# jzombie/rust-llkv

Measured on AMD Instinct MI355X. Metric: rows/sec + HBM GB/s, TPC-H Q1/Q6 SF10 at 1/2/4/8 MI355X, higher is better.
Workload: dtype f64

## Files before the change

### rust-llkv_amd/csrc/fused_scan.hip.h

```cpp
#pragma once

#ifndef __HIPCC_RTC__
#include <hip/hip_runtime.h>
#include <stdint.h>
#endif

#include "scan_params.h"
#include "planvalue_rules.h"

namespace llkv {

__device__ __forceinline__ uint64_t lane_identity(int op) {
  switch (op) {
  case OP_MIN_I64: return 0x7FFFFFFFFFFFFFFFull;
  case OP_MAX_I64: return 0x8000000000000000ull;
  default: return 0ull;
  }
}

__device__ __forceinline__ uint64_t lane_combine(int op, uint64_t a, uint64_t b) {
  const uint64_t fadd = (uint64_t)__double_as_longlong(__longlong_as_double((long long)a) + __longlong_as_double((long long)b));
  const uint64_t iadd = a + b;
  const bool lt = (int64_t)b < (int64_t)a;
  const uint64_t imin = lt ? b : a;
  const uint64_t imax = (int64_t)b > (int64_t)a ? b : a;
  const uint64_t umax = b > a ? b : a;
  return op == OP_ADD_F64 ? fadd : op == OP_ADD_I64 ? iadd : op == OP_MIN_I64 ? imin : op == OP_MAX_I64 ? imax : umax;
}

template <int OP> __device__ __forceinline__ uint64_t lane_combine_s(uint64_t a, uint64_t b) {
  if constexpr (OP == OP_ADD_F64) return (uint64_t)__double_as_longlong(__longlong_as_double((long long)a) + __longlong_as_double((long long)b));
  else if constexpr (OP == OP_ADD_I64) return a + b;
  else if constexpr (OP == OP_MIN_I64) return (int64_t)b < (int64_t)a ? b : a;
  else if constexpr (OP == OP_MAX_I64) return (int64_t)b > (int64_t)a ? b : a;
  else return b > a ? b : a;
}

template <int OP> constexpr uint64_t lane_identity_s() {
  return OP == OP_MIN_I64 ? 0x7FFFFFFFFFFFFFFFull : OP == OP_MAX_I64 ? 0x8000000000000000ull : 0ull;
}

struct I32 { using T = int32_t; static constexpr int W = 4; static constexpr bool is_float = false; };
struct U32 { using T = uint32_t; static constexpr int W = 4; static constexpr bool is_float = false; };
struct F32 { using T = float; static constexpr int W = 4; static constexpr bool is_float = true; };
struct I64 { using T = int64_t; static constexpr int W = 8; static constexpr bool is_float = false; };
struct U64 { using T = uint64_t; static constexpr int W = 8; static constexpr bool is_float = false; };
struct F64 { using T = double; static constexpr int W = 8; static constexpr bool is_float = true; };
struct I128 { using T = __int128; static constexpr int W = 16; static constexpr bool is_float = false; };
struct U8 { using T = uint8_t; static constexpr int W = 1; static constexpr bool is_float = false; };
template <class Ty, int N_> struct D8 { using T = typename Ty::T; static constexpr int W = 1; static constexpr int N = N_; static constexpr bool is_float = Ty::is_float; };

template <class... Ts> struct Cols { static constexpr int N = sizeof...(Ts); };

template <int I, class L> struct ColAt;
template <int I, class T0, class... Ts> struct ColAt<I, Cols<T0, Ts...>> { using type = typename ColAt<I - 1, Cols<Ts...>>::type; };
template <class T0, class... Ts> struct ColAt<0, Cols<T0, Ts...>> { using type = T0; };

struct Loaded {
  uint32_t w[kMaxCols][4];
};

#ifndef LLKV_NT_LOADS
#define LLKV_NT_LOADS 1
#endif
template <class V> __device__ __forceinline__ V stream_load(const V *ptr) {
#if LLKV_NT_LOADS
  return __builtin_nontemporal_load(ptr);
#else
  return *ptr;
#endif
}

template <class Ty> __device__ __forceinline__ void load_pair(const void *base, uint64_t row, uint32_t (&w)[4]) {
  if constexpr (Ty::W == 8) {
    typedef uint32_t v4u __attribute__((ext_vector_type(4)));
    const v4u v = stream_load(reinterpret_cast<const v4u *>(static_cast<const char *>(base) + row * 8));
    w[0] = v.x; w[1] = v.y; w[2] = v.z; w[3] = v.w;
  } else if constexpr (Ty::W == 4) {
    typedef uint32_t v2u __attribute__((ext_vector_type(2)));
    const v2u v = stream_load(reinterpret_cast<const v2u *>(static_cast<const char *>(base) + row * 4));
    w[0] = v.x; w[1] = v.y;
  } else {
    w[0] = stream_load(reinterpret_cast<const uint16_t *>(static_cast<const char *>(base) + row));
  }
}

template <class Ty> __device__ __forceinline__ void load_quad(const void *base, uint64_t row, uint32_t (&w)[4]) {
  static_assert(Ty::W <= 4, "four rows of an 8-byte column do not fit a column's registers");
  if constexpr (Ty::W == 4) {
    typedef uint32_t v4u __attribute__((ext_vector_type(4)));
    const v4u v = stream_load(reinterpret_cast<const v4u *>(static_cast<const char *>(base) + row * 4));
    w[0] = v.x; w[1] = v.y; w[2] = v.z; w[3] = v.w;
  } else {
    w[0] = stream_load(reinterpret_cast<const uint32_t *>(static_cast<const char *>(base) + row));
  }
}
template <class CL, int LO, int HI> __device__ __forceinline__ void load_quad_range(const ScanParams &p, uint64_t row, Loaded &ld) {
  if constexpr (LO < HI && LO < CL::N) {
    load_quad<typename ColAt<LO, CL>::type>(p.col[LO], row, ld.w[LO]);
    load_quad_range<CL, LO + 1, HI>(p, row, ld);
  }
}
template <class CL, int LO, int HI> constexpr bool cols_narrow() {
  if constexpr (LO < HI && LO < CL::N) return ColAt<LO, CL>::type::W <= 4 && ColAt<LO, CL>::type::W != 2 && cols_narrow<CL, LO + 1, HI>();
  else return true;
}

template <class CL, int I = 0> __device__ __forceinline__ void load_all(const ScanParams &p, uint64_t row, Loaded &ld) {
  if constexpr (I < CL::N) {
    load_pair<typename ColAt<I, CL>::type>(p.col[I], row, ld.w[I]);
    load_all<CL, I + 1>(p, row, ld);
  }
}

template <class CL, int LO, int HI> __device__ __forceinline__ void load_range(const ScanParams &p, uint64_t row, Loaded &ld) {
  if constexpr (LO < HI && LO < CL::N) {
    load_pair<typename ColAt<LO, CL>::type>(p.col[LO], row, ld.w[LO]);
    load_range<CL, LO + 1, HI>(p, row, ld);
  }
}

template <class Ty> struct CodedSize { static constexpr int N = 0; };
template <class Ty, int M> struct CodedSize<D8<Ty, M>> {
  static_assert(M >= 1 && M <= 256 && (M & (M - 1)) == 0 && Ty::W == 8, "a decode table has a power of two ≤ 256 of 8-byte entries");
  static constexpr int N = M;
};
template <class CL, int LO, int HI> constexpr int coded_entries() {
  if constexpr (LO < HI && LO < CL::N) return CodedSize<typename ColAt<LO, CL>::type>::N + coded_entries<CL, LO + 1, HI>();
  else return 0;
}
template <int NT> struct ValueTables {
  static __device__ __forceinline__ uint64_t *lds() { __shared__ uint64_t t[NT]; return t; }
};
template <> struct ValueTables<0> {
  static __device__ __forceinline__ uint64_t *lds() { return nullptr; }
};
template <class CL> __device__ __forceinline__ const uint64_t *stage_value_tables(const ScanParams &p) {
  constexpr int NT = coded_entries<CL, 0, CL::N>();
  uint64_t *t = ValueTables<NT>::lds();
  if constexpr (NT > 0) {
    for (uint32_t i = threadIdx.x; i < (uint32_t)NT; i += blockDim.x) t[i] = p.value_tables[i];
    __syncthreads();
  }
  return t;
}
template <class CL, int LO, int HI> __device__ __forceinline__ void decode_range(const uint64_t *vtab, Loaded &ld) {
  if constexpr (LO < HI && LO < CL::N) {
    constexpr int n = CodedSize<typename ColAt<LO, CL>::type>::N;
    if constexpr (n > 0) {
      const uint64_t *t = vtab + coded_entries<CL, 0, LO>();
      const uint32_t codes = ld.w[LO][0];
      const uint64_t a = t[codes & (uint32_t)(n - 1)], b = t[(codes >> 8) & (uint32_t)(n - 1)];
      ld.w[LO][0] = (uint32_t)a; ld.w[LO][1] = (uint32_t)(a >> 32);
      ld.w[LO][2] = (uint32_t)b; ld.w[LO][3] = (uint32_t)(b >> 32);
    }
    decode_range<CL, LO + 1, HI>(vtab, ld);
  }
}

struct Ctx {
  const ScanParams &p;
  const Loaded &ld;
  uint32_t err;
  uint64_t row;
  uint32_t perr;
  uint64_t dval;
  uint32_t dhead;

  template <class Ty> __device__ __forceinline__ typename Ty::T get(int s, int j) const {
    if constexpr (Ty::W == 8) {
      const uint64_t bits = ((uint64_t)ld.w[s][2 * j + 1] << 32) | ld.w[s][2 * j];
      if constexpr (Ty::is_float) return __longlong_as_double((long long)bits);
      else return (typename Ty::T)bits;
    } else if constexpr (Ty::W == 4) {
      if constexpr (Ty::is_float) return __uint_as_float(ld.w[s][j]);
      else return (typename Ty::T)ld.w[s][j];
    } else {
      return (uint8_t)((ld.w[s][0] >> (8 * j)) & 0xffu);
    }
  }
};

template <int S, class Ty> struct Col {
  using Type = Ty;
  static __device__ __forceinline__ typename Ty::T eval(Ctx &c, int j) { return c.get<Ty>(S, j); }
  static __device__ __forceinline__ bool valid(Ctx &, int) { return true; }
};
template <int S, class Ty, int SV> struct ColN {
  using Type = Ty;
  static __device__ __forceinline__ typename Ty::T eval(Ctx &c, int j) { return c.get<Ty>(S, j); }
  static __device__ __forceinline__ bool valid(Ctx &c, int j) { return c.get<U8>(SV, j) != 0; }
};
template <int K> struct LitI {
  using Type = I64;
  static __device__ __forceinline__ int64_t eval(Ctx &c, int) { return c.p.lit_i[K]; }
  static __device__ __forceinline__ bool valid(Ctx &, int) { return true; }
};
template <int K> struct LitU {
  using Type = U64;
  static __device__ __forceinline__ uint64_t eval(Ctx &c, int) { return (uint64_t)c.p.lit_i[K]; }
  static __device__ __forceinline__ bool valid(Ctx &, int) { return true; }
};
template <int K> struct LitF {
  using Type = F64;
  static __device__ __forceinline__ double eval(Ctx &c, int) { return c.p.lit_f[K]; }
  static __device__ __forceinline__ bool valid(Ctx &, int) { return true; }
};
template <int S> struct DictNum {
  using Type = F64;
  static __device__ __forceinline__ double eval(Ctx &c, int j) { return c.p.dict_num[S * 256 + (int)c.get<U8>(S, j)]; }
  static __device__ __forceinline__ bool valid(Ctx &, int) { return true; }
};
template <class E> struct ToF64 {
  using Type = F64;
  static __device__ __forceinline__ double eval(Ctx &c, int j) { return (double)E::eval(c, j); }
  static __device__ __forceinline__ bool valid(Ctx &c, int j) { return E::valid(c, j); }
};
template <class E> struct Widen128 {
  using Type = I128;
  static __device__ __forceinline__ __int128 eval(Ctx &c, int j) { return (__int128)(int64_t)E::eval(c, j); }
  static __device__ __forceinline__ bool valid(Ctx &c, int j) { return E::valid(c, j); }
};
template <int SLO, int SHI> struct Join128 {
  using Type = I128;
  static __device__ __forceinline__ __int128 eval(Ctx &c, int j) { return ((__int128)c.get<I64>(SHI, j) << 64) | (__int128)(unsigned __int128)c.get<U64>(SLO, j); }
  static __device__ __forceinline__ bool valid(Ctx &, int) { return true; }
};
template <class E> struct ToI64 {
  using Type = I64;
  static __device__ __forceinline__ int64_t eval(Ctx &c, int j) { return (int64_t)E::eval(c, j); }
  static __device__ __forceinline__ bool valid(Ctx &c, int j) { return E::valid(c, j); }
};

__device__ __forceinline__ int64_t f64_as_i64_sat(double x) {
  if (x != x) return 0;
  if (x >= 9223372036854775808.0) return 0x7FFFFFFFFFFFFFFFll;
  if (x <= -9223372036854775808.0) return (int64_t)0x8000000000000000ull;
  return (int64_t)x;
}

#ifndef LLKV_FIRST_ONLY_MODE
#define LLKV_FIRST_ONLY_MODE 0
#endif
enum BinKind : int { B_ADD = 1, B_SUB = 2, B_MUL = 3, B_REM = 4 };
constexpr uint32_t kErrOverflow = 1u, kErrDivZero = 2u;

__device__ __forceinline__ double f64_result_as_sse2(double r, double a, double b) {
  if (r == r) return r;
  const long long quiet = 0x0008000000000000ll;
  if (a != a) return __longlong_as_double(__double_as_longlong(a) | quiet);
  if (b != b) return __longlong_as_double(__double_as_longlong(b) | quiet);
  return __longlong_as_double((long long)0xFFF8000000000000ull);
}

template <int OP, class L, class R, int EXACT_NAN = 0> struct Bin {
  using Type = typename L::Type;
  static __device__ __forceinline__ bool valid(Ctx &c, int j) { return L::valid(c, j) & R::valid(c, j); }
  static __device__ __forceinline__ typename Type::T eval(Ctx &c, int j) {
    const auto a = L::eval(c, j);
    const auto b = R::eval(c, j);
    if constexpr (Type::is_float) {
      double r;
      if constexpr (OP == B_ADD) r = a + b;
      else if constexpr (OP == B_SUB) r = a - b;
      else if constexpr (OP == B_MUL) r = a * b;
      else r = fmod(a, b);
      if constexpr (EXACT_NAN) return f64_result_as_sse2(r, a, b);
      else return r;
    } else if constexpr (OP == B_REM) {
      const bool ok = valid(c, j);
      const int64_t x = (int64_t)a, y = (int64_t)b;
      const bool zero = y == 0;
      c.err = max(c.err, (ok & zero) ? kErrDivZero : 0u);
      return (zero | (y == -1)) ? 0 : x % y;
    } else {
      int64_t z;
      bool o;
      if constexpr (OP == B_ADD) o = __builtin_add_overflow((int64_t)a, (int64_t)b, &z);
      else if constexpr (OP == B_SUB) o = __builtin_sub_overflow((int64_t)a, (int64_t)b, &z);
      else o = __builtin_mul_overflow((int64_t)a, (int64_t)b, &z);
      c.err = max(c.err, (o & valid(c, j)) ? kErrOverflow : 0u);
      return z;
    }
  }
};
template <class E, int SIGNED> struct Fit32 {
  using Type = I64;
  static __device__ __forceinline__ bool valid(Ctx &c, int j) { return E::valid(c, j); }
  static __device__ __forceinline__ int64_t eval(Ctx &c, int j) {
    const int64_t z = (int64_t)E::eval(c, j);
    const bool fits = SIGNED ? (z >= -2147483648ll && z <= 2147483647ll) : (z >= 0 && z <= 4294967295ll);
    c.err = max(c.err, (!fits & E::valid(c, j)) ? kErrOverflow : 0u);
    return z;
  }
};
template <class E, class T32> struct Narrow32 {
  using Type = T32;
  static __device__ __forceinline__ bool valid(Ctx &c, int j) { return E::valid(c, j); }
  static __device__ __forceinline__ typename T32::T eval(Ctx &c, int j) { return (typename T32::T)E::eval(c, j); }
};
template <class L, class R> using Add = Bin<B_ADD, L, R>;
template <class L, class R> using Sub = Bin<B_SUB, L, R>;
template <class L, class R> using Mul = Bin<B_MUL, L, R>;

template <class L, class R, int EXACT_NAN = 0> struct Div {
  using Type = typename L::Type;
  static __device__ __forceinline__ bool nonzero(typename Type::T b) {
    if constexpr (Type::is_float) return __double_as_longlong(b) != 0;
    else return b != 0;
// ... 729 lines not shown
            const int op = ops.v[gg * K + k];
            const uint64_t x = sel ? contrib[k] : lane_identity(op);
            acc[gg][k] = lane_combine(op, acc[gg][k], x);
          }
        }
      }
    }
  }

  const uint32_t slot = tid + (tid >> 4);
  const uint32_t ri = tid >> 4;
  const uint32_t rq = tid & 15;
#pragma unroll
  for (int base = 0; base < LANES; base += kRedBatch) {
#pragma unroll
    for (int i = 0; i < kRedBatch; ++i) {
      const int lane = base + i;
      if (lane < LANES) {
        uint64_t v;
        if (lane == NG * K) v = err;
        else v = acc[lane / K][lane % K];
        red[i][slot] = v;
      }
    }
    __syncthreads();
    const int lane = base + (int)ri;
    if (lane < LANES) {
      const int op = ops.v[lane];
      const uint32_t seg = rq * 17;
      uint64_t v = red[ri][seg];
#pragma unroll
      for (int e = 1; e < 16; ++e) v = lane_combine(op, v, red[ri][seg + e]);
#pragma unroll
      for (int off = 8; off >= 1; off >>= 1) {
        const uint32_t lo = __shfl_xor((uint32_t)v, off, 16);
        const uint32_t hi = __shfl_xor((uint32_t)(v >> 32), off, 16);
        const uint64_t o = ((uint64_t)hi << 32) | lo;
        v = (rq & off) ? lane_combine(op, o, v) : lane_combine(op, v, o);
      }
      if (rq == 0) publish_partial(p, lane, v, tile, p.n_tiles);
    }
    __syncthreads();
  }
  }
}


template <int OP> __device__ __forceinline__ void lds_accumulate(uint64_t *slot, uint64_t x) {
  if constexpr (OP == OP_ADD_F64)
    (void)__hip_atomic_fetch_add(reinterpret_cast<double *>(slot), __longlong_as_double((long long)x), __ATOMIC_RELAXED, __HIP_MEMORY_SCOPE_WORKGROUP);
  else if constexpr (OP == OP_ADD_I64)
    (void)__hip_atomic_fetch_add(reinterpret_cast<unsigned long long *>(slot), (unsigned long long)x, __ATOMIC_RELAXED, __HIP_MEMORY_SCOPE_WORKGROUP);
  else if constexpr (OP == OP_MIN_I64)
    (void)__hip_atomic_fetch_min(reinterpret_cast<long long *>(slot), (long long)x, __ATOMIC_RELAXED, __HIP_MEMORY_SCOPE_WORKGROUP);
  else if constexpr (OP == OP_MAX_I64)
    (void)__hip_atomic_fetch_max(reinterpret_cast<long long *>(slot), (long long)x, __ATOMIC_RELAXED, __HIP_MEMORY_SCOPE_WORKGROUP);
  else
    (void)__hip_atomic_fetch_max(reinterpret_cast<unsigned long long *>(slot), (unsigned long long)x, __ATOMIC_RELAXED, __HIP_MEMORY_SCOPE_WORKGROUP);
}

template <class P, int K0 = 0> __device__ __forceinline__ void lds_accumulate_row(uint64_t *group_base, const uint64_t *contrib, uint32_t gid, uint64_t *seen) {
  if constexpr (K0 < P::K) {
    if constexpr (plan_lane_first_only<P>(K0)) {
      constexpr int i = plan_first_only_index<P>(K0);
      const uint64_t bit = 1ull << gid;
      if (!(seen[i] & bit) && contrib[K0] != lane_identity_s<plan_lane_op<P>(K0)>()) {
        lds_accumulate<plan_lane_op<P>(K0)>(group_base + K0 * kBlock, contrib[K0]);
        seen[i] |= bit;
      }
    } else {
      lds_accumulate<plan_lane_op<P>(K0)>(group_base + K0 * kBlock, contrib[K0]);
    }
    lds_accumulate_row<P, K0 + 1>(group_base, contrib, gid, seen);
  }
}

__device__ __forceinline__ void wave_lds_sync() {
  __builtin_amdgcn_fence(__ATOMIC_RELEASE, "wavefront");
  __builtin_amdgcn_wave_barrier();
  __builtin_amdgcn_fence(__ATOMIC_ACQUIRE, "wavefront");
}

__device__ __forceinline__ TileDesc load_tile_desc(const TileDesc *tiles, uint32_t i) {
  typedef const __attribute__((address_space(4))) uint64_t *ConstU64;
  ConstU64 q = (ConstU64)(unsigned long long)(tiles + i);
  TileDesc d;
  d.dev_row = q[0];
  d.logical_row = q[1];
  const uint64_t w = q[2];
  d.rows = (uint32_t)w;
  d.octant = (uint32_t)(w >> 32);
  return d;
}

constexpr int kLdsParts = kBlock / 64;

template <class P, int OP> struct OpSlots {
  int n;
  int v[P::K];
  constexpr OpSlots() : n(0), v{} {
    for (int k = 0; k < P::K; ++k)
      if (plan_lane_op<P>(k) == OP) v[n++] = k;
  }
};

template <class P, int OP>
__device__ __forceinline__ void wave_reduce_class(const ScanParams &p, const uint64_t (*acc)[kBlock], uint32_t wave, uint32_t li, uint32_t sq, uint32_t part, uint32_t n_parts) {
  constexpr OpSlots<P, OP> cls{};
  if constexpr (cls.n > 0) {
    constexpr int total = P::NG * cls.n;
#pragma unroll 1
    for (int base = 0; base < total; base += 16) {
      const int idx = base + (int)li;
      if (idx < total) {
        const int g = idx / cls.n, j = idx % cls.n;
        int k = cls.v[0];
#pragma unroll
        for (int t = 1; t < cls.n; ++t) k = j == t ? cls.v[t] : k;
        const int lane = g * P::K + k;
        const uint64_t *seg = &acc[lane][wave * 64 + sq * 16];
        uint64_t x[16];
#pragma unroll
        for (int e = 0; e < 16; ++e) x[e] = seg[(li + e) & 15];
        uint64_t v = x[0];
#pragma unroll
        for (int e = 1; e < 16; ++e) v = lane_combine_s<OP>(v, x[e]);
#pragma unroll
        for (int off = 2; off >= 1; off >>= 1) {
          const uint32_t lo = __shfl_xor((uint32_t)v, off, 4);
          const uint32_t hi = __shfl_xor((uint32_t)(v >> 32), off, 4);
          const uint64_t o = ((uint64_t)hi << 32) | lo;
          v = (sq & off) ? lane_combine_s<OP>(o, v) : lane_combine_s<OP>(v, o);
        }
        if (sq == 0) publish_partial(p, lane, v, part, n_parts);
      }
    }
  }
}

template <class P>
__device__ __forceinline__ void wave_reduce_image(const ScanParams &p, const uint64_t (*acc)[kBlock], uint32_t wave, uint32_t wl, uint32_t part, uint32_t n_parts, uint32_t err) {
  const uint32_t li = wl >> 2, sq = wl & 3;
  wave_lds_sync();
  wave_reduce_class<P, OP_ADD_F64>(p, acc, wave, li, sq, part, n_parts);
  wave_reduce_class<P, OP_ADD_I64>(p, acc, wave, li, sq, part, n_parts);
  wave_reduce_class<P, OP_MIN_I64>(p, acc, wave, li, sq, part, n_parts);
  wave_reduce_class<P, OP_MAX_I64>(p, acc, wave, li, sq, part, n_parts);
  wave_reduce_class<P, OP_MAX_U64>(p, acc, wave, li, sq, part, n_parts);
  const uint32_t wave_err = (__builtin_amdgcn_ballot_w64((err & 1u) != 0) ? 1u : 0u) | (__builtin_amdgcn_ballot_w64((err & 2u) != 0) ? 2u : 0u);
  if (wl == 0) publish_partial(p, P::NG * P::K, wave_err, part, n_parts);
  wave_lds_sync();
}

template <class P> __device__ __forceinline__ void fused_scan_body_lds(const ScanParams &p) {
  constexpr int NG = P::NG, K = P::K, U = P::U;
  constexpr LaneOpTable<P> ops{};
  __shared__ uint64_t acc[NG * K][kBlock];

  const uint32_t tid = threadIdx.x, wave = tid >> 6, wl = tid & 63;
  piggyback_fold<P>(p);

  uint32_t tile = (uint32_t)((uint64_t)blockIdx.x * p.n_tiles / gridDim.x);
  const uint32_t tile_end = (uint32_t)((uint64_t)(blockIdx.x + 1) * p.n_tiles / gridDim.x);
  if (tile >= tile_end) return;
  const uint64_t *vtab = stage_value_tables<typename P::ColList>(p);
  const uint32_t n_parts = p.n_tiles * kLdsParts;
#pragma unroll
  for (int l = 0; l < NG * K; ++l) acc[l][tid] = lane_identity(ops.v[l]);
  uint32_t err = 0, done_err = 0, done_tile = 0;
  constexpr int n_first_only = plan_first_only_index<P>(K);
  static_assert(n_first_only == 0 || NG <= 64, "the first-only masks hold one bit per group");
  uint64_t seen[n_first_only > 0 ? n_first_only : 1] = {};
  bool fresh = false;

  TileDesc td = load_tile_desc(p.tiles, tile);
  TileDesc td_next = load_tile_desc(p.tiles, tile + 1 < tile_end ? tile + 1 : tile);
  uint32_t nsteps = (td.rows + kStepRows - 1) / kStepRows;
  uint32_t s = 0;
  for (;;) {
    Loaded ld[U];
#pragma unroll
    for (int u = 0; u < U; ++u) load_all<typename P::ColList>(p, td.dev_row + (uint64_t)(s + u) * kStepRows + (uint64_t)tid * kRowsPerThread, ld[u]);
    if (fresh) {
      wave_reduce_image<P>(p, acc, wave, wl, done_tile * kLdsParts + wave, n_parts, done_err);
#pragma unroll
      for (int l = 0; l < NG * K; ++l) acc[l][tid] = lane_identity(ops.v[l]);
#pragma unroll
      for (int i = 0; i < (n_first_only > 0 ? n_first_only : 1); ++i) seen[i] = 0;
      fresh = false;
    }
#pragma unroll
    for (int u = 0; u < U; ++u) {
      decode_range<typename P::ColList, 0, P::ColList::N>(vtab, ld[u]);
      const uint32_t row0 = (s + u) * kStepRows + tid * kRowsPerThread;
#pragma unroll
      for (int j = 0; j < kRowsPerThread; ++j) {
        Ctx c{p, ld[u], 0u, td.logical_row + row0 + j};
        const bool in_tile = (row0 + j) < td.rows;
        const bool pass = in_tile & P::Pred::eval(c, j);
        uint32_t gid = P::KeyT::gid(c, j);
        gid = gid < (uint32_t)NG ? gid : 0u;
        uint64_t contrib[K];
        contrib[0] = 1;
        if constexpr (P::first) contrib[1] = c.row;
        AggOps<typename P::AggT>::contrib(c, j, contrib + P::BASE);
        err |= (pass ? c.err : 0u) | (in_tile ? c.perr : 0u);
        if (pass) lds_accumulate_row<P>(&acc[gid * K][tid], contrib, gid, seen);
      }
    }
    s += U;
    if (s >= nsteps) {
      done_tile = tile;
      done_err = err;
      err = 0;
      fresh = true;
      if (++tile >= tile_end) break;
      td = td_next;
      nsteps = (td.rows + kStepRows - 1) / kStepRows;
      s = 0;
      if (tile + 1 < tile_end) td_next = load_tile_desc(p.tiles, tile + 1);
    }
  }
  wave_reduce_image<P>(p, acc, wave, wl, done_tile * kLdsParts + wave, n_parts, done_err);
}

constexpr int kImgBlock = 1024;
constexpr int kImgStepRows = kImgBlock * kRowsPerThread;

constexpr int image_replicas(int cells, int cell_bytes = 8) {
  int r = 1;
  while (r < 32 && (long)(2 * r) * cells * cell_bytes <= 64 * 1024) r *= 2;
  return r;
}
template <bool NARROW> struct ImageCell { using T = uint64_t; };
template <> struct ImageCell<true> { using T = uint32_t; };
template <int OP> __device__ __forceinline__ void lds_accumulate(uint32_t *slot, uint64_t x) {
  static_assert(OP == OP_ADD_I64 || OP == OP_MIN_I64, "4-byte image cells hold counts, bounded integer sums and first rows");
  if constexpr (OP == OP_ADD_I64) (void)__hip_atomic_fetch_add(slot, (uint32_t)x, __ATOMIC_RELAXED, __HIP_MEMORY_SCOPE_WORKGROUP);
  else (void)__hip_atomic_fetch_min(slot, (uint32_t)x, __ATOMIC_RELAXED, __HIP_MEMORY_SCOPE_WORKGROUP);
}
template <class P, int NGS, int K0 = 0, class Cell> __device__ __forceinline__ void image_accumulate_row(Cell *img, uint32_t gid, const uint64_t *contrib) {
  if constexpr (K0 < P::K) {
    lds_accumulate<plan_lane_op<P>(K0)>(img + K0 * NGS + gid, contrib[K0]);
    image_accumulate_row<P, NGS, K0 + 1>(img, gid, contrib);
  }
}

template <class P> __device__ __forceinline__ void image_scan_body(const ScanParams &p) {
  constexpr int K = P::K, U = P::U;
  constexpr int NG = (P::NG + P::PASSES - 1) / P::PASSES;
  using Cell = typename ImageCell<P::CELL32>::T;
  constexpr int R = image_replicas(K * NG, (int)sizeof(Cell));
  __shared__ Cell img_all[R * K * NG];
  __shared__ uint32_t block_err;

  const uint32_t tid = threadIdx.x;
  Cell *img = img_all + (tid % (uint32_t)R) * (uint32_t)(K * NG);
  for (uint32_t i = tid; i < (uint32_t)(R * K * NG); i += kImgBlock) {
    const int op = plan_lane_op<P>((int)((i % (uint32_t)(K * NG)) / NG));
    if constexpr (P::CELL32) img_all[i] = op == OP_MIN_I64 ? 0xFFFFFFFFu : 0u;
    else img_all[i] = lane_identity(op);
  }
  if (tid == 0) block_err = 0;
  const uint64_t *vtab = stage_value_tables<typename P::ColList>(p);
  __syncthreads();

  uint32_t err = 0;
  auto issue = [&](const TileDesc &td, Loaded (&ld)[U]) {
#pragma unroll
    for (int u = 0; u < U; ++u) load_all<typename P::ColList>(p, td.dev_row + (uint64_t)u * kImgStepRows + (uint64_t)tid * kRowsPerThread, ld[u]);
  };
  auto accumulate = [&](const TileDesc &td, Loaded (&ld)[U]) {
#pragma unroll
    for (int u = 0; u < U; ++u) {
      decode_range<typename P::ColList, 0, P::ColList::N>(vtab, ld[u]);
      const uint32_t row0 = u * kImgStepRows + tid * kRowsPerThread;
#pragma unroll
      for (int j = 0; j < kRowsPerThread; ++j) {
        Ctx c{p, ld[u], 0u, td.logical_row + row0 + j};
        const bool in_tile = (row0 + j) < td.rows;
        uint32_t gid = P::KeyT::gid(c, j) - p.group_base;
        const bool mine = gid < (uint32_t)NG;
        const bool pass = in_tile & mine & P::Pred::eval(c, j);
        gid = mine ? gid : 0u;
        uint64_t contrib[K];
        contrib[0] = 1;
        if constexpr (P::first) contrib[1] = c.row;
        AggOps<typename P::AggT>::contrib(c, j, contrib + P::BASE);
        err |= (pass ? c.err : 0u) | (in_tile ? c.perr : 0u);
        if (pass) image_accumulate_row<P, NG>(img, gid, contrib);
      }
    }
  };
  const uint32_t n = p.n_tiles, g = gridDim.x;
  uint32_t ta = blockIdx.x, tb = ta + g;
  TileDesc da = load_tile_desc(p.tiles, ta < n ? ta : 0), db = load_tile_desc(p.tiles, tb < n ? tb : 0);
  Loaded la[U], lb[U];
  if (ta < n) issue(da, la);
  while (ta < n) {
    if (tb < n) issue(db, lb);
    accumulate(da, la);
    ta = tb + g;
    if (ta < n) { da = load_tile_desc(p.tiles, ta); issue(da, la); }
    if (tb < n) accumulate(db, lb);
    tb = ta + g;
    if (tb < n) db = load_tile_desc(p.tiles, tb);
  }
  if (err) atomicOr(&block_err, err);
  __syncthreads();
  uint64_t *out = p.tile_partials + (uint64_t)blockIdx.x * (uint64_t)(K * NG + 1);
  for (uint32_t i = tid; i < (uint32_t)(K * NG); i += kImgBlock) {
    const int op = plan_lane_op<P>((int)(i / NG));
    if constexpr (P::CELL32) {
      uint32_t v = img_all[i];
#pragma unroll 1
      for (int r = 1; r < R; ++r) {
        const uint32_t o = img_all[(uint32_t)r * (uint32_t)(K * NG) + i];
        v = op == OP_MIN_I64 ? (o < v ? o : v) : v + o;
      }
      out[i] = op == OP_MIN_I64 ? (v == 0xFFFFFFFFu ? lane_identity(OP_MIN_I64) : (uint64_t)v) : (uint64_t)(int64_t)(int32_t)v;
    } else {
      uint64_t v = img_all[i];
      if constexpr (R > 1) {
#pragma unroll 1
        for (int r = 1; r < R; ++r) v = lane_combine(op, v, img_all[(uint32_t)r * (uint32_t)(K * NG) + i]);
      }
      out[i] = v;
    }
  }
  if (tid == 0) out[K * NG] = block_err;
}
// ... 367 lines not shown
```

### rust-llkv_amd/csrc/jit.cpp

```cpp
#include "engine.hpp"

#include <hip/hiprtc.h>

#include <algorithm>
#include <chrono>
#include <cstdio>
#include <cstring>
#include <dirent.h>
#include <dlfcn.h>
#include <fstream>
#include <sys/stat.h>
#include <unistd.h>
#include <unordered_map>

namespace llkv {

#include "fused_scan_source.inc"

namespace {
std::mutex g_jit_mu;
std::unordered_map<std::string, JitKernel> g_jit_cache;
uint64_t g_jit_compiled = 0, g_jit_from_cache = 0, g_jit_from_seed = 0;

const char *kind_name(JitKind k) { return k == JitKind::Scan ? "scan" : k == JitKind::Select ? "select" : k == JitKind::Project ? "project" : k == JitKind::Probe ? "probe" : k == JitKind::Reduce ? "reduce" : k == JitKind::Image ? "image" : k == JitKind::KeyBits ? "keybits" : k == JitKind::Part ? "part" : "emit"; }
// ... 1 lines not shown
std::string wrapper_source(JitKind kind, const std::string &ts) {
  std::string s = "\nusing namespace llkv;\n";
  switch (kind) {
  case JitKind::Scan:
    s += "extern \"C\" __global__ __launch_bounds__(256) void llkv_jit_a(const ScanParams p) { fused_scan_body<" + ts + ">(p); }\n";
    break;
  case JitKind::KeyBits:
    s += "extern \"C\" __global__ __launch_bounds__(256) void llkv_jit_a(const ScanParams p) { keybits_body<" + ts + ">(p); }\n";
    break;
  case JitKind::Image:
    s += "extern \"C\" __global__ __launch_bounds__(1024) void llkv_jit_a(const ScanParams p) { image_scan_body<" + ts + ">(p); }\n";
    break;
  case JitKind::Part:
    if (ts.size() > 6 && ts.compare(ts.size() - 6, 6, ";lines") == 0)
      s += "extern \"C\" __global__ __launch_bounds__(1024) void llkv_jit_a(const ScanParams p) { part_scatter_body<" + ts.substr(0, ts.size() - 6) + ", 1024, true>(p); }\n";
    else
      s += "extern \"C\" __global__ __launch_bounds__(" + std::to_string(part_block_threads()) + ") void llkv_jit_a(const ScanParams p) { part_scatter_body<" + ts + ", " +
           std::to_string(part_block_threads()) + ">(p); }\n";
    break;
  case JitKind::Select:
    s += "extern \"C\" __global__ __launch_bounds__(256) void llkv_jit_a(const ScanParams p) { select_body<" + ts + ", false>(p); }\n";
    s += "extern \"C\" __global__ __launch_bounds__(256) void llkv_jit_b(const ScanParams p) { select_body<" + ts + ", true>(p); }\n";
    break;
  case JitKind::Project:
    s += "extern \"C\" __global__ __launch_bounds__(256) void llkv_jit_a(const ProjParams p) { project_body<" + ts + ">(p); }\n";
    break;
  case JitKind::Reduce:
    s += "extern \"C\" __global__ __launch_bounds__(256) void llkv_jit_a(const ReduceParams p) { group_reduce_body<" + ts + ">(p); }\n";
    s += "extern \"C\" __global__ __launch_bounds__(256) void llkv_jit_b(const ReduceParams p) { group_reduce_body<" + ts + ",8>(p); }\n";
    break;
  case JitKind::Emit:
    s += "extern \"C\" __global__ __launch_bounds__(256) void llkv_jit_a(const ScanParams p) { emit_body<" + ts + ", false>(p); }\n";
    s += "extern \"C\" __global__ __launch_bounds__(256) void llkv_jit_b(const ScanParams p) { emit_body<" + ts + ", true>(p); }\n";
    break;
  case JitKind::Probe:
    s += "extern \"C\" __global__ __launch_bounds__(256) void llkv_jit_a(const ScanParams p) { probe_emit_body<" + ts + ", false>(p); }\n";
    s += "extern \"C\" __global__ __launch_bounds__(256) void llkv_jit_b(const ScanParams p) { probe_emit_body<" + ts + ", true>(p); }\n";
    break;
  }
  return s;
}

uint64_t fnv1a(const std::string &s) {
  uint64_t h = 0xcbf29ce484222325ull;
  for (unsigned char c : s) h = (h ^ c) * 0x100000001b3ull;
  return h;
}

std::string cache_dir() {
  if (const char *e = std::getenv("LLKV_HIP_CACHE_DIR")) return e;
  if (const char *h = std::getenv("HOME")) if (*h) return std::string(h) + "/.cache/llkv_hip";
  return "";
}

bool private_dir(const std::string &dir) {
  if (dir.empty()) return false;
  for (size_t i = 1; i <= dir.size(); ++i)
    if (i == dir.size() || dir[i] == '/') (void)::mkdir(dir.substr(0, i).c_str(), 0700);
  struct stat st;
  if (::stat(dir.c_str(), &st) != 0 || !S_ISDIR(st.st_mode)) return false;
  return st.st_uid == ::geteuid() && (st.st_mode & 022) == 0;
}

std::string seed_dir() {
  Dl_info info;
  if (!dladdr(reinterpret_cast<const void *>(&seed_dir), &info) || !info.dli_fname) return "";
  const std::string lib = info.dli_fname;
  const size_t cut = lib.rfind('/');
  return cut == std::string::npos ? "" : lib.substr(0, cut) + "/jit_seed";
}

std::string compile_identity() {
  int major = 0, minor = 0;
  (void)hiprtcVersion(&major, &minor);
  const char *extra = std::getenv("LLKV_HIP_JIT_DEFINES");
  return "hiprtc " + std::to_string(major) + "." + std::to_string(minor) + " --offload-arch=gfx950 -O3 -std=c++17 " + (extra ? extra : "");
}

int compile_to_code(const std::string &src, std::vector<char> *code, std::string *err) {
  hiprtcProgram prog = nullptr;
  if (hiprtcCreateProgram(&prog, src.c_str(), "llkv_jit.hip", 0, nullptr, nullptr) != HIPRTC_SUCCESS) {
    *err = "hiprtcCreateProgram failed";
    return LLKV_INTERNAL;
  }
  std::vector<const char *> opts = {"--offload-arch=gfx950", "-O3", "-std=c++17"};
  std::string extra = std::getenv("LLKV_HIP_JIT_DEFINES") ? std::getenv("LLKV_HIP_JIT_DEFINES") : "";
  std::vector<std::string> extra_opts;
  for (size_t b = 0; b < extra.size();) {
    size_t e = extra.find(' ', b);
    if (e == std::string::npos) e = extra.size();
    if (e > b) extra_opts.push_back(extra.substr(b, e - b));
    b = e + 1;
  }
  for (auto &o : extra_opts) opts.push_back(o.c_str());
  hiprtcResult r = hiprtcCompileProgram(prog, (int)opts.size(), opts.data());
  if (r != HIPRTC_SUCCESS) {
    size_t n = 0;
    hiprtcGetProgramLogSize(prog, &n);
    std::string log(n, '\0');
    if (n) hiprtcGetProgramLog(prog, &log[0]);
    hiprtcDestroyProgram(&prog);
    *err = "hiprtc compile failed:\n" + log;
    return LLKV_INTERNAL;
  }
  size_t code_size = 0;
  hiprtcGetCodeSize(prog, &code_size);
  code->resize(code_size);
  hiprtcGetCode(prog, code->data());
  hiprtcDestroyProgram(&prog);
  return LLKV_OK;
}
}

static const char kBlobMagic[8] = {'L', 'L', 'K', 'V', 'J', 'I', 'T', '1'};
static uint64_t fnv1a_alt(const std::string &s) {
  uint64_t h = 0x84222325cbf29ce4ull ^ (uint64_t)s.size();
  for (unsigned char c : s) h = (h ^ c) * 0x100000001b3ull + 0x9E3779B97F4A7C15ull;
  return h;
}
static std::string blob_identity(JitKind kind, const std::string &type_string, const std::string &src) {
  char h2[32];
  std::snprintf(h2, sizeof h2, "%016llx", (unsigned long long)fnv1a_alt(src));
  return std::string(kind_name(kind)) + "|" + type_string + "\n" + h2 + "\n" + compile_identity();
}
static void blob_append_identity(std::vector<char> *file, const std::string &id) {
  file->insert(file->end(), id.begin(), id.end());
  const uint64_t n = id.size();
  file->insert(file->end(), reinterpret_cast<const char *>(&n), reinterpret_cast<const char *>(&n) + 8);
  file->insert(file->end(), kBlobMagic, kBlobMagic + 8);
}
static bool blob_take_identity(std::vector<char> *file, const std::string *expect, std::string *id_out = nullptr) {
  if (file->size() < 16 || std::memcmp(file->data() + file->size() - 8, kBlobMagic, 8) != 0) return false;
  uint64_t n = 0;
  std::memcpy(&n, file->data() + file->size() - 16, 8);
  if (n > file->size() - 16) return false;
  const std::string id(file->data() + file->size() - 16 - n, (size_t)n);
  if (expect && id != *expect) return false;
  if (id_out) *id_out = id;
  file->resize(file->size() - 16 - (size_t)n);
  return true;
}
static bool trusted_dir(const std::string &dir) {
  struct stat st;
  if (dir.empty() || ::stat(dir.c_str(), &st) != 0 || !S_ISDIR(st.st_mode)) return false;
  const bool ok = (st.st_uid == ::geteuid() || st.st_uid == 0) && (st.st_mode & 022) == 0;
  if (!ok && std::getenv("LLKV_HIP_TRACE"))
    std::fprintf(stderr, "[llkv_hip] jit: seed directory %s is ignored (owner %u, mode %o: it must belong to this user or root and be writable by its owner only — chmod 755)\n",
                 dir.c_str(), (unsigned)st.st_uid, (unsigned)(st.st_mode & 07777));
  return ok;
}

int jit_compile(JitKind kind, const std::string &type_string, JitKernel *out, std::string *err) {
  std::lock_guard<std::mutex> lk(g_jit_mu);
  const std::string key = std::string(kind_name(kind)) + "|" + type_string;
  auto it = g_jit_cache.find(key);
  if (it != g_jit_cache.end()) { *out = it->second; return LLKV_OK; }

  const std::string src = std::string(kFusedScanSource) + wrapper_source(kind, type_string);
  char hex[32];
  std::snprintf(hex, sizeof hex, "%016llx", (unsigned long long)fnv1a(src + "\n// " + compile_identity()));
  const std::string dir = cache_dir();
  const bool cacheable = private_dir(dir);
  const std::string path = dir + "/" + hex + ".hsaco";
  const bool two = kind == JitKind::Select || kind == JitKind::Probe || kind == JitKind::Emit || kind == JitKind::Reduce;
  JitKernel k;
  auto load = [&](const std::vector<char> &code, std::string *why) -> bool {
    k = JitKernel{};
    hipError_t e = hipModuleLoadData(&k.module, code.data());
    if (e != hipSuccess) { *why = std::string("hipModuleLoadData: ") + hipGetErrorString(e); return false; }
    e = hipModuleGetFunction(&k.fn, k.module, "llkv_jit_a");
    if (e == hipSuccess && two) e = hipModuleGetFunction(&k.fn2, k.module, "llkv_jit_b");
    if (e != hipSuccess) {
      *why = std::string("hipModuleGetFunction: ") + hipGetErrorString(e);
      (void)hipModuleUnload(k.module);
      return false;
    }
    return true;
  };
  std::vector<char> code;
  bool loaded = false;
  const std::string identity = blob_identity(kind, type_string, src);
  if (cacheable) {
    std::ifstream f(path, std::ios::binary);
    if (f) code.assign(std::istreambuf_iterator<char>(f), std::istreambuf_iterator<char>());
    std::string why;
    if (!code.empty() && !(blob_take_identity(&code, &identity) && (loaded = load(code, &why)))) {
      (void)::unlink(path.c_str());
      code.clear();
    }
    g_jit_from_cache += loaded ? 1 : 0;
  }
  if (!loaded && !std::getenv("LLKV_HIP_NO_JIT_SEED")) {
    static const std::string seeds = trusted_dir(seed_dir()) ? seed_dir() : std::string();
    if (!seeds.empty()) {
      std::ifstream f(seeds + "/" + hex + ".hsaco", std::ios::binary);
      if (f) code.assign(std::istreambuf_iterator<char>(f), std::istreambuf_iterator<char>());
      std::string why;
      if (!code.empty() && !(blob_take_identity(&code, &identity) && (loaded = load(code, &why)))) code.clear();
      g_jit_from_seed += loaded ? 1 : 0;
    }
  }
  if (!loaded) {
    int rc = compile_to_code(src, &code, err);
    if (rc) { *err = "plan " + type_string + ": " + *err; return rc; }
    if (cacheable) {
      const std::string tmp = path + ".tmp" + std::to_string((long)::getpid());
      std::ofstream f(tmp, std::ios::binary);
      std::vector<char> file = code;
      blob_append_identity(&file, identity);
      if (f) { f.write(file.data(), (std::streamsize)file.size()); f.close(); std::rename(tmp.c_str(), path.c_str()); }
    }
    if (!load(code, err)) return LLKV_INTERNAL;
    ++g_jit_compiled;
  }
  g_jit_cache.emplace(key, k);
  *out = k;
  return LLKV_OK;
}

int jit_launch_raw(hipFunction_t fn, uint32_t grid, void *params, size_t , hipStream_t stream, uint32_t block) {
  if (grid == 0) return LLKV_OK;
  void *args[] = {params};
  hipError_t e = hipModuleLaunchKernel(fn, grid, 1, 1, block, 1, 1, 0, stream, args, nullptr);
  if (e != hipSuccess) return set_error(LLKV_INTERNAL, std::string("hipModuleLaunchKernel: ") + hipGetErrorString(e));
  return LLKV_OK;
}

int jit_launch(const JitKernel &k, const ScanParams &p, hipStream_t stream) {
  ScanParams copy = p;
  return jit_launch_raw(k.fn, p.scan_grid ? p.scan_grid : p.n_tiles, &copy, sizeof copy, stream);
}

void jit_shutdown() {
  std::lock_guard<std::mutex> lk(g_jit_mu);
  for (auto &kv : g_jit_cache) if (kv.second.module) (void)hipModuleUnload(kv.second.module);
  g_jit_cache.clear();
}

extern "C" void llkv_hip_jit_stats(uint64_t *compiled, uint64_t *from_cache, uint64_t *from_seed) {
  std::lock_guard<std::mutex> lk(g_jit_mu);
  if (compiled) *compiled = g_jit_compiled;
  if (from_cache) *from_cache = g_jit_from_cache;
  if (from_seed) *from_seed = g_jit_from_seed;
}

extern "C" int llkv_hip_jit_verify_dir(const char *dir, uint32_t every, uint64_t *checked, uint64_t *bad, char *first_bad, uint64_t first_bad_cap) {
  if (checked) *checked = 0;
  if (bad) *bad = 0;
  if (first_bad && first_bad_cap) first_bad[0] = 0;
  if (!dir) return LLKV_INVALID_ARGUMENT;
  std::vector<std::string> names;
  if (DIR *d = ::opendir(dir)) {
    while (struct dirent *e = ::readdir(d)) {
      const std::string n = e->d_name;
      if (n.size() > 6 && n.compare(n.size() - 6, 6, ".hsaco") == 0) names.push_back(n);
    }
    ::closedir(d);
  } else {
    return LLKV_NOT_FOUND;
  }
  std::sort(names.begin(), names.end());
  if (every == 0) every = 1;
  for (size_t i = 0; i < names.size(); i += every) {
    std::ifstream f(std::string(dir) + "/" + names[i], std::ios::binary);
    std::vector<char> file((std::istreambuf_iterator<char>(f)), std::istreambuf_iterator<char>());
    std::string id;
    bool ok = blob_take_identity(&file, nullptr, &id);
    if (ok) {
      const size_t bar = id.find('|'), nl = id.find('\n');
      ok = bar != std::string::npos && nl != std::string::npos && bar < nl;
      if (ok) {
        const std::string kind_s = id.substr(0, bar), ts = id.substr(bar + 1, nl - bar - 1);
        int kind = -1;
        for (int k = 0; k <= 8; ++k) if (kind_s == kind_name((JitKind)k)) kind = k;
        ok = kind >= 0;
        if (ok) {
          const std::string src = std::string(kFusedScanSource) + wrapper_source((JitKind)kind, ts);
          char hex[32];
          std::snprintf(hex, sizeof hex, "%016llx", (unsigned long long)fnv1a(src + "\n// " + compile_identity()));
          std::vector<char> code;
          std::string err;
          ok = names[i] == std::string(hex) + ".hsaco" && id == blob_identity((JitKind)kind, ts, src) && compile_to_code(src, &code, &err) == LLKV_OK && code == file;
        }
      }
    }
    if (checked) ++*checked;
    if (!ok) {
      if (bad) ++*bad;
      if (first_bad && first_bad_cap && !first_bad[0]) std::snprintf(first_bad, (size_t)first_bad_cap, "%s", names[i].c_str());
    }
  }
  return LLKV_OK;
}

extern "C" int llkv_hip_jit_rebuild_dir(const char *from, const char *to, uint32_t shard, uint32_t n_shards, uint64_t *built, uint64_t *failed) {
  if (built) *built = 0;
  if (failed) *failed = 0;
  if (!from || !to || n_shards == 0) return LLKV_INVALID_ARGUMENT;
  std::vector<std::string> names;
  if (DIR *d = ::opendir(from)) {
    while (struct dirent *e = ::readdir(d)) {
      const std::string n = e->d_name;
      if (n.size() > 6 && n.compare(n.size() - 6, 6, ".hsaco") == 0) names.push_back(n);
    }
    ::closedir(d);
  } else {
    return LLKV_NOT_FOUND;
// ... 125 lines not shown
```

Baseline: 344.9 billion.

## Double-buffer column loads across step groups in LDS fused scan with decode tables

Adds a software-pipelined path to the LDS-accumulator fused scan. While the current group of steps is decoded and accumulated, the next group's column data is already being loaded from memory. It applies only to plans that have dictionary-coded columns, whose LDS footprint limits occupancy, and whose staged register count stays within a budget. Single-byte columns are staged as 16-bit loads and widened later, and decoded values are pinned in VGPRs to stop the compiler from rematerialising the table lookups. The aim is to hide HBM latency when low occupancy leaves too few waves to cover it, at the cost of more register pressure. A JIT define environment variable is also added to the cache key.

```diff
diff --git a/rust-llkv_amd/csrc/fused_scan.hip.h b/rust-llkv_amd/csrc/fused_scan.hip.h
--- a/rust-llkv_amd/csrc/fused_scan.hip.h
+++ b/rust-llkv_amd/csrc/fused_scan.hip.h
@@ -129,6 +129,13 @@
   if constexpr (LO < HI && LO < CL::N) return CodedSize<typename ColAt<LO, CL>::type>::N + coded_entries<CL, LO + 1, HI>();
   else return 0;
 }
+template <class CL, int LO, int HI> constexpr int step_dwords(bool decoded) {
+  if constexpr (LO < HI && LO < CL::N) {
+    using Ty = typename ColAt<LO, CL>::type;
+    const int own = (decoded && CodedSize<Ty>::N > 0) ? 4 : Ty::W == 8 ? 4 : Ty::W == 4 ? 2 : 1;
+    return own + step_dwords<CL, LO + 1, HI>(decoded);
+  } else return 0;
+}
 template <int NT> struct ValueTables {
   static __device__ __forceinline__ uint64_t *lds() { __shared__ uint64_t t[NT]; return t; }
 };
@@ -155,6 +162,32 @@
       ld.w[LO][2] = (uint32_t)b; ld.w[LO][3] = (uint32_t)(b >> 32);
     }
     decode_range<CL, LO + 1, HI>(vtab, ld);
+  }
+}
+struct Staged {
+  Loaded ld;
+  uint16_t h[kMaxCols];
+};
+template <class CL, int I = 0> __device__ __forceinline__ void stage_all(const ScanParams &p, uint64_t row, Staged &st) {
+  if constexpr (I < CL::N) {
+    if constexpr (ColAt<I, CL>::type::W == 1) st.h[I] = stream_load(reinterpret_cast<const uint16_t *>(static_cast<const char *>(p.col[I]) + row));
+    else load_pair<typename ColAt<I, CL>::type>(p.col[I], row, st.ld.w[I]);
+    stage_all<CL, I + 1>(p, row, st);
+  }
+}
+template <class CL, int I = 0> __device__ __forceinline__ void widen_staged(Staged &st) {
+  if constexpr (I < CL::N) {
+    if constexpr (ColAt<I, CL>::type::W == 1) st.ld.w[I][0] = st.h[I];
+    widen_staged<CL, I + 1>(st);
+  }
+}
+template <class CL, int LO, int HI> __device__ __forceinline__ void pin_decoded(Loaded &ld) {
+  if constexpr (LO < HI && LO < CL::N) {
+    if constexpr (CodedSize<typename ColAt<LO, CL>::type>::N > 0) {
+#pragma unroll
+      for (int i = 0; i < 4; ++i) asm volatile("" : "+v"(ld.w[LO][i]));
+    }
+    pin_decoded<CL, LO + 1, HI>(ld);
   }
 }
 
@@ -1190,6 +1223,18 @@
   wave_lds_sync();
 }
 
+#ifndef LLKV_SCAN_PREFETCH
+#define LLKV_SCAN_PREFETCH 1
+#endif
+template <class P> constexpr bool scan_prefetch_plan() {
+  using CL = typename P::ColList;
+  constexpr int tables = coded_entries<CL, 0, CL::N>();
+  constexpr long lds_bytes = (long)P::NG * P::K * kBlock * 8 + (long)tables * 8;
+  constexpr int staged = P::U * (step_dwords<CL, 0, CL::N>(true) + step_dwords<CL, 0, CL::N>(false));
+  constexpr int per_cu_limit = LLKV_SCAN_PREFETCH >= 2 ? 3 : 2;
+  return LLKV_SCAN_PREFETCH != 0 && tables > 0 && per_cu_limit * lds_bytes > 160l * 1024 && staged <= 144;
+}
+
 template <class P> __device__ __forceinline__ void fused_scan_body_lds(const ScanParams &p) {
   constexpr int NG = P::NG, K = P::K, U = P::U;
   constexpr LaneOpTable<P> ops{};
@@ -1215,6 +1260,69 @@
   TileDesc td_next = load_tile_desc(p.tiles, tile + 1 < tile_end ? tile + 1 : tile);
   uint32_t nsteps = (td.rows + kStepRows - 1) / kStepRows;
   uint32_t s = 0;
+  if constexpr (scan_prefetch_plan<P>()) {
+    auto group = [&](Staged(&cur)[U], Staged(&nxt)[U]) __attribute__((always_inline)) -> bool {
+      const bool tile_ends = s + U >= nsteps, scan_ends = tile_ends && tile + 1 >= tile_end;
+      const uint64_t next_row = scan_ends ? td.dev_row + (uint64_t)s * kStepRows : tile_ends ? td_next.dev_row : td.dev_row + (uint64_t)(s + U) * kStepRows;
+#pragma unroll
+      for (int u = 0; u < U; ++u) stage_all<typename P::ColList>(p, next_row + (uint64_t)u * kStepRows + (uint64_t)tid * kRowsPerThread, nxt[u]);
+      if (fresh) {
+        wave_reduce_image<P>(p, acc, wave, wl, done_tile * kLdsParts + wave, n_parts, done_err);
+#pragma unroll
+        for (int l = 0; l < NG * K; ++l) acc[l][tid] = lane_identity(ops.v[l]);
+#pragma unroll
+        for (int i = 0; i < (n_first_only > 0 ? n_first_only : 1); ++i) seen[i] = 0;
+        fresh = false;
+      }
+#pragma unroll
+      for (int u = 0; u < U; ++u) {
+        widen_staged<typename P::ColList>(cur[u]);
+        decode_range<typename P::ColList, 0, P::ColList::N>(vtab, cur[u].ld);
+      }
+#pragma unroll
+      for (int u = 0; u < U; ++u) pin_decoded<typename P::ColList, 0, P::ColList::N>(cur[u].ld);
+#pragma unroll
+      for (int u = 0; u < U; ++u) {
+        const uint32_t row0 = (s + u) * kStepRows + tid * kRowsPerThread;
+#pragma unroll
+        for (int j = 0; j < kRowsPerThread; ++j) {
+          Ctx c{p, cur[u].ld, 0u, td.logical_row + row0 + j};
+          const bool in_tile = (row0 + j) < td.rows;
+          const bool pass = in_tile & P::Pred::eval(c, j);
+          uint32_t gid = P::KeyT::gid(c, j);
+          gid = gid < (uint32_t)NG ? gid : 0u;
+          uint64_t contrib[K];
+          contrib[0] = 1;
+          if constexpr (P::first) contrib[1] = c.row;
+          AggOps<typename P::AggT>::contrib(c, j, contrib + P::BASE);
+          err |= (pass ? c.err : 0u) | (in_tile ? c.perr : 0u);
+          if (pass) lds_accumulate_row<P>(&acc[gid * K][tid], contrib, gid, seen);
+        }
+      }
+      s += U;
+      if (s >= nsteps) {
+        done_tile = tile;
+        done_err = err;
+        err = 0;
+        fresh = true;
+        if (++tile >= tile_end) return true;
+        td = td_next;
+        nsteps = (td.rows + kStepRows - 1) / kStepRows;
+        s = 0;
+        if (tile + 1 < tile_end) td_next = load_tile_desc(p.tiles, tile + 1);
+      }
+      return false;
+    };
+    Staged la[U], lb[U];
+#pragma unroll
+    for (int u = 0; u < U; ++u) stage_all<typename P::ColList>(p, td.dev_row + (uint64_t)u * kStepRows + (uint64_t)tid * kRowsPerThread, la[u]);
+    for (;;) {
+      if (group(la, lb)) break;
+      if (group(lb, la)) break;
+    }
+    wave_reduce_image<P>(p, acc, wave, wl, done_tile * kLdsParts + wave, n_parts, done_err);
+    return;
+  }
   for (;;) {
     Loaded ld[U];
 #pragma unroll
diff --git a/rust-llkv_amd/csrc/jit.cpp b/rust-llkv_amd/csrc/jit.cpp
--- a/rust-llkv_amd/csrc/jit.cpp
+++ b/rust-llkv_amd/csrc/jit.cpp
@@ -177,7 +177,8 @@
 
 int jit_compile(JitKind kind, const std::string &type_string, JitKernel *out, std::string *err) {
   std::lock_guard<std::mutex> lk(g_jit_mu);
-  const std::string key = std::string(kind_name(kind)) + "|" + type_string;
+  const char *defines = std::getenv("LLKV_HIP_JIT_DEFINES");
+  const std::string key = std::string(kind_name(kind)) + "|" + type_string + (defines && *defines ? std::string("\n") + defines : std::string());
   auto it = g_jit_cache.find(key);
   if (it != g_jit_cache.end()) { *out = it->second; return LLKV_OK; }
 
```

Result: no change. 344.5 billion, median of 2 (-0.1%).
